# boelnasr/ManipulaPy

Hardware: AMD Instinct MI355X
Metric: joint-timesteps/sec (NxBxDOF) inverse-dynamics trajectory (higher is better)
Workload: dtype f32; 1 GPU; UR5 6-DOF, B=4096 x N=1000, inverse_dynamics_trajectory fp32 (BASELINE configs[1]); robot=ur5, dof=6, B_per_gpu=4096, N=1000, rows_per_gpu=4096000, op=id, inputs=q/qd/qdd histories resident in HBM, input_sets=3, bytes_between_reuse=1179648000, kernel_variant=robot-specialised (hiprtc)

## Files before the change

### manipulapy_amd/csrc/mp_core.h

```cpp
#pragma once

#if !defined(__HIPCC_RTC__)
#include <cmath>
#endif

#include "mp_model.h"

#if defined(__HIPCC__) || defined(__HIPCC_RTC__)
#define MP_HD __host__ __device__ __forceinline__
#else
#define MP_HD inline
#endif

#if defined(__clang__)
#define MP_HAS_PACKED 1
typedef float mp_f2 __attribute__((ext_vector_type(2)));
typedef int mp_i2 __attribute__((ext_vector_type(2)));
typedef unsigned mp_u2 __attribute__((ext_vector_type(2)));
#endif

template <typename T> struct MpTraits;
template <> struct MpTraits<float> {
  using S = float;
  static MP_HD float splat(float v) { return v; }
// ... 54 lines not shown
  c = __builtin_bit_cast(double, __builtin_bit_cast(unsigned long long, b) ^ ((unsigned long long)((qs + 0x40000000u) & 0x80000000u) << 32));
}
#if MP_HAS_PACKED
MP_HD void mp_sincos(mp_f2 x, mp_f2& s, mp_f2& c) {
  const mp_f2 kf = __builtin_elementwise_fma(x, (mp_f2)(0.636619772367581343f), (mp_f2)(12582912.0f));
  const mp_f2 k = kf - 12582912.0f;
  mp_f2 r = __builtin_elementwise_fma(-k, (mp_f2)(1.57079637050628662109375f), x);
  r = __builtin_elementwise_fma(-k, (mp_f2)(-4.37113900018624283e-8f), r);
  const mp_f2 r2 = r * r;
  mp_f2 ps = __builtin_elementwise_fma(r2, (mp_f2)(-1.9515295891e-4f), (mp_f2)(8.3321608736e-3f));
  ps = __builtin_elementwise_fma(r2, ps, (mp_f2)(-1.6666654611e-1f));
  ps = __builtin_elementwise_fma(r * r2, ps, r);
  mp_f2 pc = __builtin_elementwise_fma(r2, (mp_f2)(2.443315711809948e-5f), (mp_f2)(-1.388731625493765e-3f));
  pc = __builtin_elementwise_fma(r2, pc, (mp_f2)(4.166664568298827e-2f));
  pc = __builtin_elementwise_fma(r2 * r2, pc, __builtin_elementwise_fma(r2, (mp_f2)(-0.5f), (mp_f2)(1.0f)));
  const mp_i2 q = __builtin_bit_cast(mp_i2, kf);
  const mp_i2 odd = (q & 1) != 0;
  const mp_f2 a = odd ? pc : ps;
  const mp_f2 b = odd ? ps : pc;
  const mp_u2 qs = __builtin_bit_cast(mp_u2, q) << 30;
  s = __builtin_bit_cast(mp_f2, __builtin_bit_cast(mp_u2, a) ^ (qs & 0x80000000u));
  c = __builtin_bit_cast(mp_f2, __builtin_bit_cast(mp_u2, b) ^ ((qs + 0x40000000u) & 0x80000000u));
}
#endif

MP_HD float mp_min(float a, float b) { return a < b ? a : b; }
MP_HD float mp_max(float a, float b) { return a > b ? a : b; }
MP_HD double mp_min(double a, double b) { return a < b ? a : b; }
MP_HD double mp_max(double a, double b) { return a > b ? a : b; }
#if MP_HAS_PACKED
MP_HD mp_f2 mp_min(mp_f2 a, mp_f2 b) { return (a < b) ? a : b; }
MP_HD mp_f2 mp_max(mp_f2 a, mp_f2 b) { return (a > b) ? a : b; }
#endif
MP_HD float mp_abs(float a) { return __builtin_fabsf(a); }
MP_HD double mp_abs(double a) { return __builtin_fabs(a); }
#if MP_HAS_PACKED
MP_HD mp_f2 mp_abs(mp_f2 a) { return __builtin_elementwise_abs(a); }
#endif
MP_HD float mp_sqrt(float x) { return sqrtf(x); }
MP_HD double mp_sqrt(double x) { return sqrt(x); }
#if MP_HAS_PACKED
MP_HD mp_f2 mp_sqrt(mp_f2 x) { return (mp_f2){sqrtf(x.x), sqrtf(x.y)}; }
#endif
MP_HD float mp_rsqrt(float x) {
#if defined(__HIP_DEVICE_COMPILE__)
  const float y = __builtin_amdgcn_rsqf(x);
  const float e = fmaf(-(x * y), y, 1.0f);
  return fmaf(0.5f * y, e, y);
#else
  return 1.0f / sqrtf(x);
#endif
}
MP_HD double mp_rsqrt(double x) { return 1.0 / sqrt(x); }
#if MP_HAS_PACKED
MP_HD mp_f2 mp_rsqrt(mp_f2 x) { return (mp_f2){mp_rsqrt(x.x), mp_rsqrt(x.y)}; }
#endif
template <typename T>
MP_HD T mp_clip(T v, typename MpTraits<T>::S lo, typename MpTraits<T>::S hi) {
  return mp_min(mp_max(v, MpTraits<T>::splat(lo)), MpTraits<T>::splat(hi));
}

MP_HD int mp_hi_word(float x) { return __builtin_bit_cast(int, x); }
MP_HD int mp_hi_word(double x) { return (int)(__builtin_bit_cast(long long, x) >> 32); }
template <typename T> struct MpBadBits;
template <> struct MpBadBits<float> { static constexpr int POS = 0x7f800000; static constexpr unsigned NEG = 0xff800000u; };
template <> struct MpBadBits<double> { static constexpr int POS = 0x7ff00000; static constexpr unsigned NEG = 0xfff00000u; };

template <typename T>
struct MpBad {
  int ms = 0;
  unsigned mu = 0;
  MP_HD void add(T v) {
    const int b = mp_hi_word(v);
    ms = b > ms ? b : ms;
    mu = (unsigned)b > mu ? (unsigned)b : mu;
  }
  template <int N> MP_HD void add(const T (&v)[N]) {
#pragma unroll
    for (int i = 0; i < N; ++i) add(v[i]);
  }
  MP_HD bool any() const { return ms >= MpBadBits<T>::POS || mu >= MpBadBits<T>::NEG; }
};
MP_HD void mp_poison_if(bool bad, float& v) {
  const unsigned b = __builtin_bit_cast(unsigned, v);
  v = __builtin_bit_cast(float, bad ? 0x7fc00000u : b);
}
MP_HD void mp_poison_if(bool bad, double& v) {
  const unsigned long long b = __builtin_bit_cast(unsigned long long, v);
  v = __builtin_bit_cast(double, bad ? 0x7ff8000000000000ull : b);
}
#if MP_HAS_PACKED
template <>
struct MpBad<mp_f2> {
  MpBad<float> x, y;
  MP_HD void add(mp_f2 v) { x.add(v.x); y.add(v.y); }
  template <int N> MP_HD void add(const mp_f2 (&v)[N]) {
#pragma unroll
    for (int i = 0; i < N; ++i) add(v[i]);
  }
};
#endif
template <typename T, int N>
MP_HD void mp_poison_if(bool bad, T (&v)[N]) {
#pragma unroll
  for (int i = 0; i < N; ++i) mp_poison_if(bad, v[i]);
}

template <typename MT>
MP_HD const auto& mp_joint_of(const MT& M, int i) { return M.j[i]; }
#if defined(__HIP_DEVICE_COMPILE__)
typedef const __attribute__((address_space(4))) MpModel<float> MpModelConstF;
typedef const __attribute__((address_space(4))) MpModel<double> MpModelConstD;
__device__ __forceinline__ const __attribute__((address_space(4))) MpJoint<float>& mp_joint_of(MpModelConstF& M, int i) {
  MpModelConstF* p = &M;
  asm volatile("" : "+s"(p));
  return p->j[i];
}
__device__ __forceinline__ const __attribute__((address_space(4))) MpJoint<double>& mp_joint_of(MpModelConstD& M, int i) {
  MpModelConstD* p = &M;
  asm volatile("" : "+s"(p));
  return p->j[i];
}
typedef const __attribute__((address_space(4))) MpModelRev<float> MpModelRevConstF;
template <> struct MpAllRevolute<MpModelRevConstF> { static constexpr bool value = true; };
template <> struct MpAllRevolute<__attribute__((address_space(4))) MpModelRev<float>> { static constexpr bool value = true; };
__device__ __forceinline__ const __attribute__((address_space(4))) MpJoint<float>& mp_joint_of(MpModelRevConstF& M, int i) {
  MpModelRevConstF* p = &M;
  asm volatile("" : "+s"(p));
  return p->j[i];
}
#endif

template <typename T, typename S>
MP_HD void mp_motion_A(S ca, S sa, S a, T& wx, T& wy, T& wz, T& vx, T& vy, T& vz) {
  const T ty = vy + a * wz, tz = vz - a * wy;
  vy = ca * ty + sa * tz;
  vz = ca * tz - sa * ty;
  const T uy = wy;
  wy = ca * uy + sa * wz;
  wz = ca * wz - sa * uy;
  (void)wx; (void)vx;
}
template <typename T>
MP_HD void mp_motion_B(T c, T s, T d, T& wx, T& wy, T& wz, T& vx, T& vy, T& vz) {
  const T tx = vx + d * wy, ty = vy - d * wx;
  vx = c * tx + s * ty;
  vy = c * ty - s * tx;
  const T ux = wx;
  wx = c * ux + s * wy;
  wy = c * wy - s * ux;
  (void)wz; (void)vz;
}
template <typename T, typename S>
MP_HD void mp_force_down_A(S ca, S sa, S a, T& nx, T& ny, T& nz, T& fx, T& fy, T& fz) {
  const T ty = ny + a * fz, tz = nz - a * fy;
  ny = ca * ty + sa * tz;
  nz = ca * tz - sa * ty;
  const T uy = fy;
  fy = ca * uy + sa * fz;
  fz = ca * fz - sa * uy;
  (void)nx; (void)fx;
}
template <typename T>
MP_HD void mp_force_down_B(T c, T s, T d, T& nx, T& ny, T& nz, T& fx, T& fy, T& fz) {
  const T tx = nx + d * fy, ty = ny - d * fx;
  nx = c * tx + s * ty;
  ny = c * ty - s * tx;
  const T ux = fx;
  fx = c * ux + s * fy;
  fy = c * fy - s * ux;
  (void)nz; (void)fz;
}
template <typename T>
MP_HD void mp_force_up_B(T c, T s, T d, T& nx, T& ny, T& nz, T& fx, T& fy, T& fz) {
  const T gx = c * fx - s * fy, gy = s * fx + c * fy;
  const T mx = c * nx - s * ny, my = s * nx + c * ny;
  fx = gx; fy = gy;
  nx = mx - d * gy;
  ny = my + d * gx;
  (void)nz; (void)fz;
}
template <typename T, typename S>
MP_HD void mp_force_up_A(S ca, S sa, S a, T& nx, T& ny, T& nz, T& fx, T& fy, T& fz) {
  const T gy = ca * fy - sa * fz, gz = sa * fy + ca * fz;
  const T my = ca * ny - sa * nz, mz = sa * ny + ca * nz;
  fy = gy; fz = gz;
  ny = my - a * gz;
  nz = mz + a * gy;
  (void)nx; (void)fx;
}

template <typename T, int N>
struct MpJointState {
  T s[N], c[N], d[N];
};

template <typename T, int N, typename MT>
MP_HD void mp_joint_state(const MT& M, const T (&q)[N], MpJointState<T, N>& js) {
  constexpr bool kAllRev = MpAllRevolute<MT>::value;
#pragma unroll
  for (int i = 0; i < N; ++i) {
    const auto& J = mp_joint_of(M, i);
    const T qr = kAllRev ? q[i] : J.rev * q[i];
    T s0, c0;
    mp_sincos(qr, s0, c0);
    js.s[i] = s0 * J.co + c0 * J.so;
    js.c[i] = c0 * J.co - s0 * J.so;
    if (kAllRev) js.d[i] = MpTraits<T>::splat(J.d);
    else js.d[i] = J.d + (q[i] - qr);
  }
}

struct MpNoScale {
  template <typename T> MP_HD void joint(int, const T&, const T&, const T&, const T&, const T&, const T&) {}
  template <typename T> MP_HD void body(int, const T&, const T&, const T&, const T&, const T&, const T&) {}
  template <typename T> MP_HD void child(int, const T&, const T&, const T&, const T&, const T&, const T&) {}
};
template <typename T, int N>
struct MpRowScale {
  static constexpr int J = N > 1 ? 1 : 0;
  static constexpr int JF = N > 2 ? 2 : N - 1;
  T bm, cm, f;
  static MP_HD T inf3(const T& x, const T& y, const T& z) { return mp_max(mp_max(mp_abs(x), mp_abs(y)), mp_abs(z)); }
  MP_HD void body(int i, const T& nx, const T& ny, const T& nz, const T&, const T&, const T&) {
    if (i == J) bm = inf3(nx, ny, nz);
  }
  MP_HD void joint(int i, const T&, const T&, const T&, const T& fx, const T& fy, const T& fz) {
    if (i == JF) f = inf3(fx, fy, fz);
  }
  MP_HD void child(int i, const T& nx, const T& ny, const T& nz, const T&, const T&, const T&) {
    if (i == J + 1) cm = inf3(nx, ny, nz);
  }
  template <typename S> MP_HD T scale(S lscale) const {
    const T lf = f * MpTraits<T>::splat(lscale);
    if (N > J + 1) return mp_max(mp_max(bm, cm), lf);
    return mp_max(bm, lf);
  }
};
template <typename T, int N, bool HAS_FTIP, typename SC, typename MT>
MP_HD void mp_rnea_impl(const MT& M, const typename MpTraits<T>::S (&a0)[3], const T (&tipn)[3], const T (&tipf)[3],
                        const MpJointState<T, N>& js, const T (&qd)[N], const T (&qdd)[N], T (&tau)[N], SC& sc) {
  using S = typename MpTraits<T>::S;
  using TR = MpTraits<T>;
  const T zero = TR::splat(S(0));
  T fnx[N], fny[N], fnz[N], ffx[N], ffy[N], ffz[N];
  T wx = zero, wy = zero, wz = zero, vx = zero, vy = zero, vz = zero;
  T dwx = zero, dwy = zero, dwz = zero, dvx = TR::splat(a0[0]), dvy = TR::splat(a0[1]), dvz = TR::splat(a0[2]);
  T tnx = zero, tny = zero, tnz = zero, tfx = zero, tfy = zero, tfz = zero;
  if (HAS_FTIP) { tnx = tipn[0]; tny = tipn[1]; tnz = tipn[2]; tfx = tipf[0]; tfy = tipf[1]; tfz = tipf[2]; }

#pragma unroll
  for (int i = 0; i < N; ++i) {
    const auto& J = mp_joint_of(M, i);
    if (i > 0) {
      mp_motion_A(J.ca, J.sa, J.a, wx, wy, wz, vx, vy, vz);
      mp_motion_A(J.ca, J.sa, J.a, dwx, dwy, dwz, dvx, dvy, dvz);
      if (HAS_FTIP) mp_force_down_A(J.ca, J.sa, J.a, tnx, tny, tnz, tfx, tfy, tfz);
    }
    const T c = js.c[i], s = js.s[i], d = js.d[i];
    mp_motion_B(c, s, d, wx, wy, wz, vx, vy, vz);
    mp_motion_B(c, s, d, dwx, dwy, dwz, dvx, dvy, dvz);
    if (HAS_FTIP) mp_force_down_B(c, s, d, tnx, tny, tnz, tfx, tfy, tfz);

    if (MpAllRevolute<MT>::value) {
      const T qdr = qd[i], ar = qdd[i];
      wz += qdr;
      dwx += qdr * wy;
      dwy -= qdr * wx;
      dwz += ar;
      dvx += qdr * vy;
      dvy -= qdr * vx;
    } else {
      const T qdr = J.rev * qd[i], qdp = qd[i] - qdr;
      const T ar = J.rev * qdd[i], ap = qdd[i] - ar;
      wz += qdr;
      vz += qdp;
      dwx += qdr * wy;
      dwy -= qdr * wx;
      dwz += ar;
      dvx += qdr * vy + qdp * wy;
      dvy -= qdr * vx + qdp * wx;
      dvz += ap;
    }

    const T pnx = J.Ixx * wx + J.Ixy * wy + J.Ixz * wz + (J.hy * vz - J.hz * vy);
    const T pny = J.Ixy * wx + J.Iyy * wy + J.Iyz * wz + (J.hz * vx - J.hx * vz);
    const T pnz = J.Ixz * wx + J.Iyz * wy + J.Izz * wz + (J.hx * vy - J.hy * vx);
    const T pfx = J.m * vx - (J.hy * wz - J.hz * wy);
    const T pfy = J.m * vy - (J.hz * wx - J.hx * wz);
    const T pfz = J.m * vz - (J.hx * wy - J.hy * wx);
    fnx[i] = J.Ixx * dwx + J.Ixy * dwy + J.Ixz * dwz + (J.hy * dvz - J.hz * dvy) + (wy * pnz - wz * pny) + (vy * pfz - vz * pfy);
    fny[i] = J.Ixy * dwx + J.Iyy * dwy + J.Iyz * dwz + (J.hz * dvx - J.hx * dvz) + (wz * pnx - wx * pnz) + (vz * pfx - vx * pfz);
    fnz[i] = J.Ixz * dwx + J.Iyz * dwy + J.Izz * dwz + (J.hx * dvy - J.hy * dvx) + (wx * pny - wy * pnx) + (vx * pfy - vy * pfx);
    ffx[i] = J.m * dvx - (J.hy * dwz - J.hz * dwy) + (wy * pfz - wz * pfy);
    ffy[i] = J.m * dvy - (J.hz * dwx - J.hx * dwz) + (wz * pfx - wx * pfz);
    ffz[i] = J.m * dvz - (J.hx * dwy - J.hy * dwx) + (wx * pfy - wy * pfx);
    sc.body(i, fnx[i], fny[i], fnz[i], ffx[i], ffy[i], ffz[i]);
  }
  if (HAS_FTIP) {
    fnx[N - 1] += tnx; fny[N - 1] += tny; fnz[N - 1] += tnz;
    ffx[N - 1] += tfx; ffy[N - 1] += tfy; ffz[N - 1] += tfz;
  }
#pragma unroll
  for (int i = N - 1; i >= 0; --i) {
    const auto& J = mp_joint_of(M, i);
    if (MpAllRevolute<MT>::value) tau[i] = fnz[i];
    else tau[i] = J.rev * fnz[i] + (S(1) - J.rev) * ffz[i];
    sc.joint(i, fnx[i], fny[i], fnz[i], ffx[i], ffy[i], ffz[i]);
    if (i > 0) {
      T nx = fnx[i], ny = fny[i], nz = fnz[i], fx = ffx[i], fy = ffy[i], fz = ffz[i];
      mp_force_up_B(js.c[i], js.s[i], js.d[i], nx, ny, nz, fx, fy, fz);
      mp_force_up_A(J.ca, J.sa, J.a, nx, ny, nz, fx, fy, fz);
      sc.child(i, nx, ny, nz, fx, fy, fz);
      fnx[i - 1] += nx; fny[i - 1] += ny; fnz[i - 1] += nz;
      ffx[i - 1] += fx; ffy[i - 1] += fy; ffz[i - 1] += fz;
    }
  }
}

template <typename T, int N, bool HAS_FTIP, typename MT>
MP_HD void mp_rnea(const MT& M, const typename MpTraits<T>::S (&a0)[3], const T (&tipn)[3], const T (&tipf)[3],
                   const MpJointState<T, N>& js, const T (&qd)[N], const T (&qdd)[N], T (&tau)[N]) {
  MpNoScale sc;
  mp_rnea_impl<T, N, HAS_FTIP>(M, a0, tipn, tipf, js, qd, qdd, tau, sc);
}

template <typename T, int N, bool HAS_FTIP, typename MT>
MP_HD void mp_rnea(const MT& M, const MpCall<typename MpTraits<T>::S>& C, const MpJointState<T, N>& js,
                   const T (&qd)[N], const T (&qdd)[N], T (&tau)[N]) {
  using TR = MpTraits<T>;
  const T tn[3] = {TR::splat(C.F1n[0]), TR::splat(C.F1n[1]), TR::splat(C.F1n[2])};
  const T tf[3] = {TR::splat(C.F1f[0]), TR::splat(C.F1f[1]), TR::splat(C.F1f[2])};
  mp_rnea<T, N, HAS_FTIP>(M, C.a0, tn, tf, js, qd, qdd, tau);
}

#ifndef MP_HARD_ROW_K
#define MP_HARD_ROW_K 8.0f
#endif
#ifndef MP_ADAPTIVE_F32
#define MP_ADAPTIVE_F32 1
#endif
template <int N>
MP_HD bool mp_id_row_is_hard(const float (&tau)[N], float scale) {
  float rowmax = mp_abs(tau[0]);
#pragma unroll
  for (int i = 1; i < N; ++i) rowmax = mp_max(rowmax, mp_abs(tau[i]));
  return scale > MP_HARD_ROW_K * rowmax;
}

template <int N, bool HAS_FTIP, typename MT>
MP_HD bool mp_rnea_f32(const MT& M, const MpCall<float>& C, const MpJointState<float, N>& js, const float (&qd)[N],
                       const float (&qdd)[N], float (&tau)[N]) {
#if MP_ADAPTIVE_F32
  const float tn[3] = {C.F1n[0], C.F1n[1], C.F1n[2]}, tf[3] = {C.F1f[0], C.F1f[1], C.F1f[2]};
  MpRowScale<float, N> sc;
  mp_rnea_impl<float, N, HAS_FTIP>(M, C.a0, tn, tf, js, qd, qdd, tau, sc);
  return mp_id_row_is_hard<N>(tau, sc.scale(M.lscale));
#else
  mp_rnea<float, N, HAS_FTIP>(M, C, js, qd, qdd, tau);
  return false;
#endif
}

template <int N> struct MpColdSlot { static constexpr int BYTES = 8 * N * 8 + 4 * N * 4; };
template <int N>
struct MpColdLocal {
  double f[8 * N];
  float j[4 * N];
  MP_HD double getf(int k) const { return f[k]; }
  MP_HD void putf(int k, double v) { f[k] = v; }
  MP_HD float getj(int k) const { return j[k]; }
  MP_HD void putj(int k, float v) { j[k] = v; }
};
#if defined(__HIP_DEVICE_COMPILE__)
#define MP_LDS_AS __attribute__((address_space(3)))
#else
#define MP_LDS_AS
#endif
template <int N>
struct MpColdMem {
  MP_LDS_AS char* p;
  MP_HD double getf(int k) const { return reinterpret_cast<const volatile MP_LDS_AS double*>(p)[k]; }
  MP_HD void putf(int k, double v) { reinterpret_cast<volatile MP_LDS_AS double*>(p)[k] = v; }
  MP_HD float getj(int k) const { return reinterpret_cast<const volatile MP_LDS_AS float*>(p + 8 * N * 8)[k]; }
  MP_HD void putj(int k, float v) { reinterpret_cast<volatile MP_LDS_AS float*>(p + 8 * N * 8)[k] = v; }
};

#if defined(__clang__)
#define MP_ROLLED _Pragma("clang loop unroll(disable)")
#else
#define MP_ROLLED
#endif
#if defined(__HIP_DEVICE_COMPILE__)
#define MP_STAGE() __builtin_amdgcn_sched_barrier(0)
#else
#define MP_STAGE() ((void)0)
#endif
template <int N, bool HAS_FTIP, typename MT, typename ST>
MP_HD void mp_rnea_cold(const MT& M, const MpCall<float>& C, const float (&q)[N], const float (&qd)[N], const float (&qdd)[N], ST st,
                        float (&tau)[N]) {
  double wx = 0, wy = 0, wz = 0, vx = 0, vy = 0, vz = 0;
  double dwx = 0, dwy = 0, dwz = 0, dvx = (double)C.a0[0], dvy = (double)C.a0[1], dvz = (double)C.a0[2];
  double tnx = 0, tny = 0, tnz = 0, tfx = 0, tfy = 0, tfz = 0;
  if (HAS_FTIP) { tnx = (double)C.F1n[0]; tny = (double)C.F1n[1]; tnz = (double)C.F1n[2]; tfx = (double)C.F1f[0]; tfy = (double)C.F1f[1]; tfz = (double)C.F1f[2]; }
#pragma unroll
  for (int i = 0; i < N; ++i) { st.putj(N + i, q[i]); st.putj(2 * N + i, qd[i]); st.putj(3 * N + i, qdd[i]); }
  MP_ROLLED
  for (int i = 0; i < N; ++i) {
    const auto& J = mp_joint_of(M, i);
    const float qi = st.getj(N + i);
    double s, c, d;
    {
      const double qr = (double)J.rev * (double)qi;
      double s0, c0;
      mp_sincos(qr, s0, c0);
      s = s0 * (double)J.co + c0 * (double)J.so;
      c = c0 * (double)J.co - s0 * (double)J.so;
      d = (double)J.d + ((double)qi - qr);
      st.putf(6 * N + i, s); st.putf(7 * N + i, c); st.putj(i, (float)d);
    }
    MP_STAGE();
    const double ca = (double)J.ca, sa = (double)J.sa, la = (double)J.a;
    if (i > 0) {
      mp_motion_A<double, double>(ca, sa, la, wx, wy, wz, vx, vy, vz);
      mp_motion_A<double, double>(ca, sa, la, dwx, dwy, dwz, dvx, dvy, dvz);
      if (HAS_FTIP) mp_force_down_A<double, double>(ca, sa, la, tnx, tny, tnz, tfx, tfy, tfz);
    }
    mp_motion_B<double>(c, s, d, wx, wy, wz, vx, vy, vz);
    mp_motion_B<double>(c, s, d, dwx, dwy, dwz, dvx, dvy, dvz);
    if (HAS_FTIP) mp_force_down_B<double>(c, s, d, tnx, tny, tnz, tfx, tfy, tfz);
    const double rev = (double)J.rev, qdi = (double)st.getj(2 * N + i), qddi = (double)st.getj(3 * N + i);
    const double qdr = rev * qdi, qdp = qdi - qdr;
    const double ar = rev * qddi, ap = qddi - ar;
    wz += qdr;
    vz += qdp;
    dwx += qdr * wy;
    dwy -= qdr * wx;
    dwz += ar;
    dvx += qdr * vy + qdp * wy;
    dvy -= qdr * vx + qdp * wx;
    dvz += ap;
    MP_STAGE();
    const double Ixx = (double)J.Ixx, Ixy = (double)J.Ixy, Ixz = (double)J.Ixz, Iyy = (double)J.Iyy, Iyz = (double)J.Iyz, Izz = (double)J.Izz;
    const double hx = (double)J.hx, hy = (double)J.hy, hz = (double)J.hz, m = (double)J.m;
    const double pnx = Ixx * wx + Ixy * wy + Ixz * wz + (hy * vz - hz * vy);
    const double pny = Ixy * wx + Iyy * wy + Iyz * wz + (hz * vx - hx * vz);
    const double pnz = Ixz * wx + Iyz * wy + Izz * wz + (hx * vy - hy * vx);
    const double pfx = m * vx - (hy * wz - hz * wy);
    const double pfy = m * vy - (hz * wx - hx * wz);
    const double pfz = m * vz - (hx * wy - hy * wx);
    MP_STAGE();
    st.putf(6 * i + 0, Ixx * dwx + Ixy * dwy + Ixz * dwz + (hy * dvz - hz * dvy) + (wy * pnz - wz * pny) + (vy * pfz - vz * pfy));
    MP_STAGE();
    st.putf(6 * i + 1, Ixy * dwx + Iyy * dwy + Iyz * dwz + (hz * dvx - hx * dvz) + (wz * pnx - wx * pnz) + (vz * pfx - vx * pfz));
    MP_STAGE();
    st.putf(6 * i + 2, Ixz * dwx + Iyz * dwy + Izz * dwz + (hx * dvy - hy * dvx) + (wx * pny - wy * pnx) + (vx * pfy - vy * pfx));
    MP_STAGE();
    st.putf(6 * i + 3, m * dvx - (hy * dwz - hz * dwy) + (wy * pfz - wz * pfy));
    st.putf(6 * i + 4, m * dvy - (hz * dwx - hx * dwz) + (wz * pfx - wx * pfz));
    st.putf(6 * i + 5, m * dvz - (hx * dwy - hy * dwx) + (wx * pfy - wy * pfx));
    MP_STAGE();
  }
  double ax = tnx, ay = tny, az = tnz, bx = tfx, by = tfy, bz = tfz;
  MP_ROLLED
  for (int i = N - 1; i >= 0; --i) {
    const auto& J = mp_joint_of(M, i);
    double nx = st.getf(6 * i + 0) + ax, ny = st.getf(6 * i + 1) + ay, nz = st.getf(6 * i + 2) + az;
    double fx = st.getf(6 * i + 3) + bx, fy = st.getf(6 * i + 4) + by, fz = st.getf(6 * i + 5) + bz;
    const double rev = (double)J.rev;
    st.putj(N + i, (float)(rev * nz + (1.0 - rev) * fz));
    if (i > 0) {
      const double s = st.getf(6 * N + i), c = st.getf(7 * N + i), d = (double)st.getj(i);
      mp_force_up_B<double>(c, s, d, nx, ny, nz, fx, fy, fz);
      mp_force_up_A<double, double>((double)J.ca, (double)J.sa, (double)J.a, nx, ny, nz, fx, fy, fz);
      ax = nx; ay = ny; az = nz; bx = fx; by = fy; bz = fz;
    }
  }
#pragma unroll
  for (int i = 0; i < N; ++i) tau[i] = st.getj(N + i);
}

template <typename T> struct MpIsF32 { static constexpr bool value = false; };
template <> struct MpIsF32<float> { static constexpr bool value = true; };
template <typename T, int N, bool HAS_FTIP, typename MT>
MP_HD void mp_rnea_row(const MT& M, const MpCall<typename MpTraits<T>::S>& C, const MpJointState<T, N>& js, const T (&q)[N],
                       const T (&qd)[N], const T (&qdd)[N], T (&tau)[N]) {
  if constexpr (MpIsF32<T>::value) {
    if (mp_rnea_f32<N, HAS_FTIP>(M, C, js, qd, qdd, tau)) {
      MpColdLocal<N> st;
      if (C.cold_model) mp_rnea_cold<N, HAS_FTIP>(*static_cast<const MpModel<double>*>(C.cold_model), C, q, qd, qdd, st, tau);
      else mp_rnea_cold<N, HAS_FTIP>(M, C, q, qd, qdd, st, tau);
    }
  } else {
    mp_rnea<T, N, HAS_FTIP>(M, C, js, qd, qdd, tau);
  }
}

template <typename T, typename MT>
MP_HD void mp_wrench_to_frame1(const MT& M, const T (&F)[6], T (&tn)[3], T (&tf)[3]) {
  const auto& R = M.base_R;
  const auto& p = M.base_p;
  const T nx = F[0] - (p[1] * F[5] - p[2] * F[4]), ny = F[1] - (p[2] * F[3] - p[0] * F[5]), nz = F[2] - (p[0] * F[4] - p[1] * F[3]);
#pragma unroll
  for (int k = 0; k < 3; ++k) {
    tn[k] = R[0 + k] * nx + R[3 + k] * ny + R[6 + k] * nz;
    tf[k] = R[0 + k] * F[3] + R[3 + k] * F[4] + R[6 + k] * F[5];
  }
}

template <typename T, int N, typename MT>
MP_HD void mp_mass_matrix(const MT& M, const MpJointState<T, N>& js, T (&Mq)[N][N]) {
  using S = typename MpTraits<T>::S;
  using TR = MpTraits<T>;
  const S a0[3] = {S(0), S(0), S(0)};
  const T zero = TR::splat(S(0));
  const T z3[3] = {zero, zero, zero};
  T col[N][N];
#pragma unroll
  for (int j = 0; j < N; ++j) {
    T qd[N], qdd[N];
#pragma unroll
    for (int k = 0; k < N; ++k) { qd[k] = zero; qdd[k] = (k == j) ? TR::splat(S(1)) : zero; }
    mp_rnea<T, N, false>(M, a0, z3, z3, js, qd, qdd, col[j]);
  }
#pragma unroll
  for (int i = 0; i < N; ++i)
#pragma unroll
    for (int j = 0; j < N; ++j) Mq[i][j] = S(0.5) * (col[j][i] + col[i][j]);
}

template <typename T>
struct MpRbi {
  T m, hx, hy, hz, xx, xy, xz, yy, yz, zz;
};

template <typename T>
MP_HD void mp_rbi_up_B(T c, T s, T d, MpRbi<T>& I) {
  const T hx = c * I.hx - s * I.hy, hy = s * I.hx + c * I.hy;
  const T cc = c * c, ss = s * s, sc = s * c;
  const T xx = cc * I.xx - (sc + sc) * I.xy + ss * I.yy;
  const T yy = ss * I.xx + (sc + sc) * I.xy + cc * I.yy;
  const T xy = sc * (I.xx - I.yy) + (cc - ss) * I.xy;
  const T xz = c * I.xz - s * I.yz, yz = s * I.xz + c * I.yz;
  const T t = d * (I.hz + I.hz) + I.m * d * d;
  I.xx = xx + t; I.yy = yy + t; I.xy = xy;
  I.xz = xz - d * hx; I.yz = yz - d * hy;
  I.hx = hx; I.hy = hy; I.hz = I.hz + I.m * d;
}
template <typename T, typename S>
MP_HD void mp_rbi_up_A(S ca, S sa, S a, MpRbi<T>& I) {
  const T hy = ca * I.hy - sa * I.hz, hz = sa * I.hy + ca * I.hz;
  const S cc = ca * ca, ss = sa * sa, sc = sa * ca;
  const T yy = cc * I.yy - (sc + sc) * I.yz + ss * I.zz;
  const T zz = ss * I.yy + (sc + sc) * I.yz + cc * I.zz;
  const T yz = sc * (I.yy - I.zz) + (cc - ss) * I.yz;
  const T xy = ca * I.xy - sa * I.xz, xz = sa * I.xy + ca * I.xz;
  const T t = a * (I.hx + I.hx) + I.m * (a * a);
  I.yy = yy + t; I.zz = zz + t; I.yz = yz;
  I.xy = xy - a * hy; I.xz = xz - a * hz;
  I.hy = hy; I.hz = hz; I.hx = I.hx + I.m * a;
}

template <typename T, int N, typename MT>
MP_HD void mp_mass_matrix_crba(const MT& M, const MpJointState<T, N>& js, T (&Mq)[N][N]) {
  using S = typename MpTraits<T>::S;
  using TR = MpTraits<T>;
  const T zero = TR::splat(S(0));
  MpRbi<T> Ic;
  Ic.m = zero; Ic.hx = zero; Ic.hy = zero; Ic.hz = zero;
  Ic.xx = zero; Ic.xy = zero; Ic.xz = zero; Ic.yy = zero; Ic.yz = zero; Ic.zz = zero;
#pragma unroll
  for (int i = N - 1; i >= 0; --i) {
    const auto& J = mp_joint_of(M, i);
    Ic.m = Ic.m + J.m; Ic.hx = Ic.hx + J.hx; Ic.hy = Ic.hy + J.hy; Ic.hz = Ic.hz + J.hz;
    Ic.xx = Ic.xx + J.Ixx; Ic.xy = Ic.xy + J.Ixy; Ic.xz = Ic.xz + J.Ixz; Ic.yy = Ic.yy + J.Iyy; Ic.yz = Ic.yz + J.Iyz;
    Ic.zz = Ic.zz + J.Izz;
    const S r = J.rev, p = S(1) - J.rev;
    T nx = r * Ic.xz + p * Ic.hy, ny = r * Ic.yz - p * Ic.hx, nz = r * Ic.zz;
    T fx = -(r * Ic.hy), fy = r * Ic.hx, fz = p * Ic.m;
    Mq[i][i] = r * nz + p * fz;
#pragma unroll
    for (int k = i; k > 0; --k) {
      const auto& Jk = mp_joint_of(M, k);
      mp_force_up_B(js.c[k], js.s[k], js.d[k], nx, ny, nz, fx, fy, fz);
      mp_force_up_A(Jk.ca, Jk.sa, Jk.a, nx, ny, nz, fx, fy, fz);
      const auto& Jp = mp_joint_of(M, k - 1);
      const T v = Jp.rev * nz + (S(1) - Jp.rev) * fz;
      Mq[k - 1][i] = v;
      Mq[i][k - 1] = v;
    }
    if (i > 0) {
      mp_rbi_up_B(js.c[i], js.s[i], js.d[i], Ic);
      mp_rbi_up_A(J.ca, J.sa, J.a, Ic);
    }
  }
}

template <typename T, int N>
MP_HD void mp_spd_solve(T (&A)[N][N], T (&b)[N]) {
#pragma unroll
  for (int j = 0; j < N; ++j) {
    T d = A[j][j];
#pragma unroll
    for (int k = 0; k < j; ++k) d -= A[j][k] * A[j][k];
    const T inv = mp_rsqrt(d);
    A[j][j] = inv;
#pragma unroll
    for (int i = j + 1; i < N; ++i) {
      T v = A[i][j];
#pragma unroll
      for (int k = 0; k < j; ++k) v -= A[i][k] * A[j][k];
      A[i][j] = v * inv;
    }
  }
#pragma unroll
  for (int i = 0; i < N; ++i) {
    T v = b[i];
#pragma unroll
    for (int k = 0; k < i; ++k) v -= A[i][k] * b[k];
    b[i] = v * A[i][i];
  }
#pragma unroll
  for (int i = N - 1; i >= 0; --i) {
    T v = b[i];
#pragma unroll
    for (int k = i + 1; k < N; ++k) v -= A[k][i] * b[k];
    b[i] = v * A[i][i];
  }
// ... 189 lines not shown
```

### manipulapy_amd/csrc/mp_dyn.h

```cpp
#pragma once

#include "mp_core.h"

#if defined(__clang__)
#define MP_NOUNROLL _Pragma("nounroll")
#else
#define MP_NOUNROLL
#endif

template <typename T, int CAP>
struct MpDynState {
  T s[CAP], c[CAP], d[CAP];
};

template <typename T, typename MT, int CAP>
MP_HD void mp_dyn_joint_state(const MT& M, int n, const T* q, MpDynState<T, CAP>& js) {
  MP_NOUNROLL
  for (int i = 0; i < n; ++i) {
    const auto& J = M.j[i];
    const T qr = J.rev * q[i];
    T s0, c0;
    mp_sincos(qr, s0, c0);
    js.s[i] = s0 * J.co + c0 * J.so;
    js.c[i] = c0 * J.co - s0 * J.so;
    js.d[i] = J.d + (q[i] - qr);
  }
}

template <typename T, bool HAS_FTIP, typename MT, int CAP>
MP_HD void mp_dyn_rnea(const MT& M, int n, const T (&a0)[3], const T (&tipn)[3], const T (&tipf)[3], const MpDynState<T, CAP>& js,
                       const T* qd, const T* qdd, T* tau, T* scale = nullptr) {
  const int sJ = n > 1 ? 1 : 0, sJF = n > 2 ? 2 : n - 1;
  T s_bm = 0, s_cm = 0, s_f = 0;
  T fnx[CAP], fny[CAP], fnz[CAP], ffx[CAP], ffy[CAP], ffz[CAP];
  T wx = 0, wy = 0, wz = 0, vx = 0, vy = 0, vz = 0;
  T dwx = 0, dwy = 0, dwz = 0, dvx = a0[0], dvy = a0[1], dvz = a0[2];
  T tnx = 0, tny = 0, tnz = 0, tfx = 0, tfy = 0, tfz = 0;
  if (HAS_FTIP) { tnx = tipn[0]; tny = tipn[1]; tnz = tipn[2]; tfx = tipf[0]; tfy = tipf[1]; tfz = tipf[2]; }
  MP_NOUNROLL
  for (int i = 0; i < n; ++i) {
    const auto& J = M.j[i];
    if (i > 0) {
      mp_motion_A(J.ca, J.sa, J.a, wx, wy, wz, vx, vy, vz);
      mp_motion_A(J.ca, J.sa, J.a, dwx, dwy, dwz, dvx, dvy, dvz);
      if (HAS_FTIP) mp_force_down_A(J.ca, J.sa, J.a, tnx, tny, tnz, tfx, tfy, tfz);
    }
    const T c = js.c[i], s = js.s[i], d = js.d[i];
    mp_motion_B(c, s, d, wx, wy, wz, vx, vy, vz);
    mp_motion_B(c, s, d, dwx, dwy, dwz, dvx, dvy, dvz);
    if (HAS_FTIP) mp_force_down_B(c, s, d, tnx, tny, tnz, tfx, tfy, tfz);
    const T qdr = J.rev * qd[i], qdp = qd[i] - qdr;
    const T ar = J.rev * qdd[i], ap = qdd[i] - ar;
    wz += qdr;
    vz += qdp;
    dwx += qdr * wy;
    dwy -= qdr * wx;
    dwz += ar;
    dvx += qdr * vy + qdp * wy;
    dvy -= qdr * vx + qdp * wx;
    dvz += ap;
    const T pnx = J.Ixx * wx + J.Ixy * wy + J.Ixz * wz + (J.hy * vz - J.hz * vy);
    const T pny = J.Ixy * wx + J.Iyy * wy + J.Iyz * wz + (J.hz * vx - J.hx * vz);
    const T pnz = J.Ixz * wx + J.Iyz * wy + J.Izz * wz + (J.hx * vy - J.hy * vx);
    const T pfx = J.m * vx - (J.hy * wz - J.hz * wy);
    const T pfy = J.m * vy - (J.hz * wx - J.hx * wz);
    const T pfz = J.m * vz - (J.hx * wy - J.hy * wx);
    fnx[i] = J.Ixx * dwx + J.Ixy * dwy + J.Ixz * dwz + (J.hy * dvz - J.hz * dvy) + (wy * pnz - wz * pny) + (vy * pfz - vz * pfy);
    fny[i] = J.Ixy * dwx + J.Iyy * dwy + J.Iyz * dwz + (J.hz * dvx - J.hx * dvz) + (wz * pnx - wx * pnz) + (vz * pfx - vx * pfz);
    fnz[i] = J.Ixz * dwx + J.Iyz * dwy + J.Izz * dwz + (J.hx * dvy - J.hy * dvx) + (wx * pny - wy * pnx) + (vx * pfy - vy * pfx);
    ffx[i] = J.m * dvx - (J.hy * dwz - J.hz * dwy) + (wy * pfz - wz * pfy);
    ffy[i] = J.m * dvy - (J.hz * dwx - J.hx * dwz) + (wz * pfx - wx * pfz);
    ffz[i] = J.m * dvz - (J.hx * dwy - J.hy * dwx) + (wx * pfy - wy * pfx);
    if (scale && i == sJ) s_bm = mp_max(mp_max(mp_abs(fnx[i]), mp_abs(fny[i])), mp_abs(fnz[i]));
  }
  if (HAS_FTIP) {
    fnx[n - 1] += tnx; fny[n - 1] += tny; fnz[n - 1] += tnz;
    ffx[n - 1] += tfx; ffy[n - 1] += tfy; ffz[n - 1] += tfz;
  }
  MP_NOUNROLL
  for (int i = n - 1; i >= 0; --i) {
    const auto& J = M.j[i];
    tau[i] = J.rev * fnz[i] + (T(1) - J.rev) * ffz[i];
    if (scale && i == sJF) s_f = mp_max(mp_max(mp_abs(ffx[i]), mp_abs(ffy[i])), mp_abs(ffz[i]));
    if (i > 0) {
      T nx = fnx[i], ny = fny[i], nz = fnz[i], fx = ffx[i], fy = ffy[i], fz = ffz[i];
      mp_force_up_B(js.c[i], js.s[i], js.d[i], nx, ny, nz, fx, fy, fz);
      mp_force_up_A(J.ca, J.sa, J.a, nx, ny, nz, fx, fy, fz);
      if (scale && i == sJ + 1) s_cm = mp_max(mp_max(mp_abs(nx), mp_abs(ny)), mp_abs(nz));
      fnx[i - 1] += nx; fny[i - 1] += ny; fnz[i - 1] += nz;
      ffx[i - 1] += fx; ffy[i - 1] += fy; ffz[i - 1] += fz;
    }
  }
  if (scale) *scale = mp_max(mp_max(s_bm, s_cm), s_f * (T)M.lscale);
}

#if defined(__HIP_DEVICE_COMPILE__)
typedef const __attribute__((address_space(4))) MpBigModel<double> MpBigConstD;
#else
typedef const MpBigModel<double> MpBigConstD;
#endif
MP_HD bool mp_dyn_row_is_hard(const float* tau, int n, float scale) {
  float rowmax = 0.0f;
  for (int i = 0; i < n; ++i) rowmax = mp_max(rowmax, mp_abs(tau[i]));
  return scale > MP_HARD_ROW_K * rowmax;
}
template <int CAP, bool HAS_FTIP>
MP_HD void mp_dyn_row_id_f64(MpBigConstD& Md, const MpCall<float>& C, const float* q, const float* qd, const float* qdd, float* tau) {
  const int n = Md.n;
  double a[CAP], b[CAP], c[CAP], t[CAP];
  for (int j = 0; j < n; ++j) { a[j] = (double)q[j]; b[j] = (double)qd[j]; c[j] = (double)qdd[j]; }
  const double a0[3] = {(double)C.a0[0], (double)C.a0[1], (double)C.a0[2]};
  const double tn[3] = {(double)C.F1n[0], (double)C.F1n[1], (double)C.F1n[2]}, tf[3] = {(double)C.F1f[0], (double)C.F1f[1], (double)C.F1f[2]};
  MpDynState<double, CAP> js;
  mp_dyn_joint_state<double>(Md, n, a, js);
  mp_dyn_rnea<double, HAS_FTIP>(Md, n, a0, tn, tf, js, b, c, t);
  for (int j = 0; j < n; ++j) tau[j] = (float)t[j];
}

template <typename T, typename MT, int CAP>
MP_HD void mp_dyn_mass_matrix(const MT& M, int n, const MpDynState<T, CAP>& js, T* Mq, int ld) {
  MpRbi<T> Ic;
  Ic.m = 0; Ic.hx = 0; Ic.hy = 0; Ic.hz = 0; Ic.xx = 0; Ic.xy = 0; Ic.xz = 0; Ic.yy = 0; Ic.yz = 0; Ic.zz = 0;
  MP_NOUNROLL
  for (int i = n - 1; i >= 0; --i) {
    const auto& J = M.j[i];
    Ic.m = Ic.m + J.m; Ic.hx = Ic.hx + J.hx; Ic.hy = Ic.hy + J.hy; Ic.hz = Ic.hz + J.hz;
    Ic.xx = Ic.xx + J.Ixx; Ic.xy = Ic.xy + J.Ixy; Ic.xz = Ic.xz + J.Ixz; Ic.yy = Ic.yy + J.Iyy; Ic.yz = Ic.yz + J.Iyz;
    Ic.zz = Ic.zz + J.Izz;
    const T r = J.rev, p = T(1) - J.rev;
    T nx = r * Ic.xz + p * Ic.hy, ny = r * Ic.yz - p * Ic.hx, nz = r * Ic.zz;
    T fx = -(r * Ic.hy), fy = r * Ic.hx, fz = p * Ic.m;
    Mq[i * ld + i] = r * nz + p * fz;
    MP_NOUNROLL
    for (int k = i; k > 0; --k) {
      const auto& Jk = M.j[k];
      mp_force_up_B(js.c[k], js.s[k], js.d[k], nx, ny, nz, fx, fy, fz);
      mp_force_up_A(Jk.ca, Jk.sa, Jk.a, nx, ny, nz, fx, fy, fz);
      const T rp = M.j[k - 1].rev;
      const T v = rp * nz + (T(1) - rp) * fz;
      Mq[(k - 1) * ld + i] = v;
      Mq[i * ld + (k - 1)] = v;
    }
    if (i > 0) {
      mp_rbi_up_B(js.c[i], js.s[i], js.d[i], Ic);
      mp_rbi_up_A(J.ca, J.sa, J.a, Ic);
    }
  }
}

template <typename T>
MP_HD void mp_dyn_spd_solve(int n, T* A, int ld, T* b) {
  MP_NOUNROLL
  for (int j = 0; j < n; ++j) {
    T d = A[j * ld + j];
    for (int k = 0; k < j; ++k) d -= A[j * ld + k] * A[j * ld + k];
    const T inv = mp_rsqrt(d);
    A[j * ld + j] = inv;
    for (int i = j + 1; i < n; ++i) {
      T v = A[i * ld + j];
      for (int k = 0; k < j; ++k) v -= A[i * ld + k] * A[j * ld + k];
      A[i * ld + j] = v * inv;
    }
  }
  MP_NOUNROLL
  for (int i = 0; i < n; ++i) {
    T v = b[i];
    for (int k = 0; k < i; ++k) v -= A[i * ld + k] * b[k];
    b[i] = v * A[i * ld + i];
  }
  MP_NOUNROLL
  for (int i = n - 1; i >= 0; --i) {
    T v = b[i];
    for (int k = i + 1; k < n; ++k) v -= A[k * ld + i] * b[k];
    b[i] = v * A[i * ld + i];
  }
}

template <int CAP, typename T, bool HAS_FTIP, typename MT>
MP_HD void mp_dyn_forward_dynamics(const MT& M, int n, const T (&a0)[3], const T (&tipn)[3], const T (&tipf)[3], const T* q,
                                   const T* qd, const T* tau, T* qdd) {
  MpDynState<T, CAP> js;
  mp_dyn_joint_state<T>(M, n, q, js);
  T zero[CAP], bias[CAP], Mq[CAP * CAP];
  for (int k = 0; k < n; ++k) zero[k] = T(0);
  mp_dyn_rnea<T, HAS_FTIP>(M, n, a0, tipn, tipf, js, qd, zero, bias);
  mp_dyn_mass_matrix<T>(M, n, js, Mq, CAP);
  for (int k = 0; k < n; ++k) qdd[k] = tau[k] - bias[k];
  mp_dyn_spd_solve<T>(n, Mq, CAP, qdd);
}

template <typename T, typename MT, int CAP>
MP_HD void mp_dyn_fk_jac(const MT& M, int n, const MpDynState<T, CAP>& js, T* Tout, T* Jout) {
  T x0 = M.base_R[0], x1 = M.base_R[3], x2 = M.base_R[6];
  T y0 = M.base_R[1], y1 = M.base_R[4], y2 = M.base_R[7];
  T z0 = M.base_R[2], z1 = M.base_R[5], z2 = M.base_R[8];
  T p0 = M.base_p[0], p1 = M.base_p[1], p2 = M.base_p[2];
  MP_NOUNROLL
  for (int i = 0; i < n; ++i) {
    const auto& J = M.j[i];
    if (i > 0) {
      p0 += J.a * x0; p1 += J.a * x1; p2 += J.a * x2;
      const T a0 = y0, a1 = y1, a2 = y2;
      y0 = J.ca * a0 + J.sa * z0; y1 = J.ca * a1 + J.sa * z1; y2 = J.ca * a2 + J.sa * z2;
      z0 = J.ca * z0 - J.sa * a0; z1 = J.ca * z1 - J.sa * a1; z2 = J.ca * z2 - J.sa * a2;
    }
    if (Jout) {
      const T cx = p1 * z2 - p2 * z1, cy = p2 * z0 - p0 * z2, cz = p0 * z1 - p1 * z0;
      const T r = J.rev, pr = T(1) - J.rev;
      Jout[0 * n + i] = r * z0; Jout[1 * n + i] = r * z1; Jout[2 * n + i] = r * z2;
      Jout[3 * n + i] = r * cx + pr * z0; Jout[4 * n + i] = r * cy + pr * z1; Jout[5 * n + i] = r * cz + pr * z2;
    }
    const T c = js.c[i], s = js.s[i], d = js.d[i];
    const T b0 = x0, b1 = x1, b2 = x2;
    x0 = c * b0 + s * y0; x1 = c * b1 + s * y1; x2 = c * b2 + s * y2;
    y0 = c * y0 - s * b0; y1 = c * y1 - s * b1; y2 = c * y2 - s * b2;
    p0 += d * z0; p1 += d * z1; p2 += d * z2;
  }
  if (Tout) {
    const auto& R = M.tool_R;
    const auto& t = M.tool_p;
    Tout[0] = x0 * R[0] + y0 * R[3] + z0 * R[6]; Tout[1] = x0 * R[1] + y0 * R[4] + z0 * R[7]; Tout[2] = x0 * R[2] + y0 * R[5] + z0 * R[8];
    Tout[4] = x1 * R[0] + y1 * R[3] + z1 * R[6]; Tout[5] = x1 * R[1] + y1 * R[4] + z1 * R[7]; Tout[6] = x1 * R[2] + y1 * R[5] + z1 * R[8];
    Tout[8] = x2 * R[0] + y2 * R[3] + z2 * R[6]; Tout[9] = x2 * R[1] + y2 * R[4] + z2 * R[7]; Tout[10] = x2 * R[2] + y2 * R[5] + z2 * R[8];
    Tout[3] = p0 + x0 * t[0] + y0 * t[1] + z0 * t[2];
    Tout[7] = p1 + x1 * t[0] + y1 * t[1] + z1 * t[2];
// ... 186 lines not shown
```

Baseline: 385.7 billion joint-timesteps/s.

## Reformulate RNEA forward pass with classical origin acceleration instead of spatial velocity

Drops the linear velocity state and tracks the classical origin acceleration directly. New combined transform helpers propagate omega, its derivative, and the linear acceleration together, and the body force formulas are simplified to avoid computing momentum terms. This cuts ALU work and register pressure in the hot per-joint loop of the specialised, cold-path and dynamic kernels. It risks small numerical differences from the reordered floating-point operations.

```diff
diff --git a/manipulapy_amd/csrc/mp_core.h b/manipulapy_amd/csrc/mp_core.h
--- a/manipulapy_amd/csrc/mp_core.h
+++ b/manipulapy_amd/csrc/mp_core.h
@@ -230,6 +230,32 @@
   (void)wz; (void)vz;
 }
 template <typename T, typename S>
+MP_HD void mp_accel_A(S ca, S sa, S l, T& wx, T& wy, T& wz, T& dwx, T& dwy, T& dwz, T& ax, T& ay, T& az) {
+  ax = ax - l * (wy * wy + wz * wz);
+  const T ty = ay + l * (dwz + wx * wy), tz = az - l * (dwy - wx * wz);
+  ay = ca * ty + sa * tz;
+  az = ca * tz - sa * ty;
+  const T ey = dwy;
+  dwy = ca * ey + sa * dwz;
+  dwz = ca * dwz - sa * ey;
+  const T uy = wy;
+  wy = ca * uy + sa * wz;
+  wz = ca * wz - sa * uy;
+}
+template <typename T>
+MP_HD void mp_accel_B(T c, T s, T d, T& wx, T& wy, T& wz, T& dwx, T& dwy, T& dwz, T& ax, T& ay, T& az) {
+  const T tx = ax + d * (dwy + wx * wz), ty = ay - d * (dwx - wy * wz);
+  az = az - d * (wx * wx + wy * wy);
+  ax = c * tx + s * ty;
+  ay = c * ty - s * tx;
+  const T ex = dwx;
+  dwx = c * ex + s * dwy;
+  dwy = c * dwy - s * ex;
+  const T ux = wx;
+  wx = c * ux + s * wy;
+  wy = c * wy - s * ux;
+}
+template <typename T, typename S>
 MP_HD void mp_force_down_A(S ca, S sa, S a, T& nx, T& ny, T& nz, T& fx, T& fy, T& fz) {
   const T ty = ny + a * fz, tz = nz - a * fy;
   ny = ca * ty + sa * tz;
@@ -322,8 +348,8 @@
   using TR = MpTraits<T>;
   const T zero = TR::splat(S(0));
   T fnx[N], fny[N], fnz[N], ffx[N], ffy[N], ffz[N];
-  T wx = zero, wy = zero, wz = zero, vx = zero, vy = zero, vz = zero;
-  T dwx = zero, dwy = zero, dwz = zero, dvx = TR::splat(a0[0]), dvy = TR::splat(a0[1]), dvz = TR::splat(a0[2]);
+  T wx = zero, wy = zero, wz = zero;
+  T dwx = zero, dwy = zero, dwz = zero, ax = TR::splat(a0[0]), ay = TR::splat(a0[1]), az = TR::splat(a0[2]);
   T tnx = zero, tny = zero, tnz = zero, tfx = zero, tfy = zero, tfz = zero;
   if (HAS_FTIP) { tnx = tipn[0]; tny = tipn[1]; tnz = tipn[2]; tfx = tipf[0]; tfy = tipf[1]; tfz = tipf[2]; }
 
@@ -331,13 +357,11 @@
   for (int i = 0; i < N; ++i) {
     const auto& J = mp_joint_of(M, i);
     if (i > 0) {
-      mp_motion_A(J.ca, J.sa, J.a, wx, wy, wz, vx, vy, vz);
-      mp_motion_A(J.ca, J.sa, J.a, dwx, dwy, dwz, dvx, dvy, dvz);
+      mp_accel_A(J.ca, J.sa, J.a, wx, wy, wz, dwx, dwy, dwz, ax, ay, az);
       if (HAS_FTIP) mp_force_down_A(J.ca, J.sa, J.a, tnx, tny, tnz, tfx, tfy, tfz);
     }
     const T c = js.c[i], s = js.s[i], d = js.d[i];
-    mp_motion_B(c, s, d, wx, wy, wz, vx, vy, vz);
-    mp_motion_B(c, s, d, dwx, dwy, dwz, dvx, dvy, dvz);
+    mp_accel_B(c, s, d, wx, wy, wz, dwx, dwy, dwz, ax, ay, az);
     if (HAS_FTIP) mp_force_down_B(c, s, d, tnx, tny, tnz, tfx, tfy, tfz);
 
     if (MpAllRevolute<MT>::value) {
@@ -346,33 +370,29 @@
       dwx += qdr * wy;
       dwy -= qdr * wx;
       dwz += ar;
-      dvx += qdr * vy;
-      dvy -= qdr * vx;
     } else {
       const T qdr = J.rev * qd[i], qdp = qd[i] - qdr;
       const T ar = J.rev * qdd[i], ap = qdd[i] - ar;
+      const T qdp2 = qdp + qdp;
       wz += qdr;
-      vz += qdp;
       dwx += qdr * wy;
       dwy -= qdr * wx;
       dwz += ar;
-      dvx += qdr * vy + qdp * wy;
-      dvy -= qdr * vx + qdp * wx;
-      dvz += ap;
-    }
-
-    const T pnx = J.Ixx * wx + J.Ixy * wy + J.Ixz * wz + (J.hy * vz - J.hz * vy);
-    const T pny = J.Ixy * wx + J.Iyy * wy + J.Iyz * wz + (J.hz * vx - J.hx * vz);
-    const T pnz = J.Ixz * wx + J.Iyz * wy + J.Izz * wz + (J.hx * vy - J.hy * vx);
-    const T pfx = J.m * vx - (J.hy * wz - J.hz * wy);
-    const T pfy = J.m * vy - (J.hz * wx - J.hx * wz);
-    const T pfz = J.m * vz - (J.hx * wy - J.hy * wx);
-    fnx[i] = J.Ixx * dwx + J.Ixy * dwy + J.Ixz * dwz + (J.hy * dvz - J.hz * dvy) + (wy * pnz - wz * pny) + (vy * pfz - vz * pfy);
-    fny[i] = J.Ixy * dwx + J.Iyy * dwy + J.Iyz * dwz + (J.hz * dvx - J.hx * dvz) + (wz * pnx - wx * pnz) + (vz * pfx - vx * pfz);
-    fnz[i] = J.Ixz * dwx + J.Iyz * dwy + J.Izz * dwz + (J.hx * dvy - J.hy * dvx) + (wx * pny - wy * pnx) + (vx * pfy - vy * pfx);
-    ffx[i] = J.m * dvx - (J.hy * dwz - J.hz * dwy) + (wy * pfz - wz * pfy);
-    ffy[i] = J.m * dvy - (J.hz * dwx - J.hx * dwz) + (wz * pfx - wx * pfz);
-    ffz[i] = J.m * dvz - (J.hx * dwy - J.hy * dwx) + (wx * pfy - wy * pfx);
+      ax += qdp2 * wy;
+      ay -= qdp2 * wx;
+      az += ap;
+    }
+
+    const T iwx = J.Ixx * wx + J.Ixy * wy + J.Ixz * wz;
+    const T iwy = J.Ixy * wx + J.Iyy * wy + J.Iyz * wz;
+    const T iwz = J.Ixz * wx + J.Iyz * wy + J.Izz * wz;
+    const T ux = J.hy * wz - J.hz * wy, uy = J.hz * wx - J.hx * wz, uz = J.hx * wy - J.hy * wx;
+    fnx[i] = J.Ixx * dwx + J.Ixy * dwy + J.Ixz * dwz + (J.hy * az - J.hz * ay) + (wy * iwz - wz * iwy);
+    fny[i] = J.Ixy * dwx + J.Iyy * dwy + J.Iyz * dwz + (J.hz * ax - J.hx * az) + (wz * iwx - wx * iwz);
+    fnz[i] = J.Ixz * dwx + J.Iyz * dwy + J.Izz * dwz + (J.hx * ay - J.hy * ax) + (wx * iwy - wy * iwx);
+    ffx[i] = J.m * ax - (J.hy * dwz - J.hz * dwy) - (wy * uz - wz * uy);
+    ffy[i] = J.m * ay - (J.hz * dwx - J.hx * dwz) - (wz * ux - wx * uz);
+    ffz[i] = J.m * az - (J.hx * dwy - J.hy * dwx) - (wx * uy - wy * ux);
     sc.body(i, fnx[i], fny[i], fnz[i], ffx[i], ffy[i], ffz[i]);
   }
   if (HAS_FTIP) {
@@ -477,8 +497,8 @@
 template <int N, bool HAS_FTIP, typename MT, typename ST>
 MP_HD void mp_rnea_cold(const MT& M, const MpCall<float>& C, const float (&q)[N], const float (&qd)[N], const float (&qdd)[N], ST st,
                         float (&tau)[N]) {
-  double wx = 0, wy = 0, wz = 0, vx = 0, vy = 0, vz = 0;
-  double dwx = 0, dwy = 0, dwz = 0, dvx = (double)C.a0[0], dvy = (double)C.a0[1], dvz = (double)C.a0[2];
+  double wx = 0, wy = 0, wz = 0, dwx = 0, dwy = 0, dwz = 0;
+  double ax = (double)C.a0[0], ay = (double)C.a0[1], az = (double)C.a0[2];
   double tnx = 0, tny = 0, tnz = 0, tfx = 0, tfy = 0, tfz = 0;
   if (HAS_FTIP) { tnx = (double)C.F1n[0]; tny = (double)C.F1n[1]; tnz = (double)C.F1n[2]; tfx = (double)C.F1f[0]; tfy = (double)C.F1f[1]; tfz = (double)C.F1f[2]; }
 #pragma unroll
@@ -500,58 +520,53 @@
     MP_STAGE();
     const double ca = (double)J.ca, sa = (double)J.sa, la = (double)J.a;
     if (i > 0) {
-      mp_motion_A<double, double>(ca, sa, la, wx, wy, wz, vx, vy, vz);
-      mp_motion_A<double, double>(ca, sa, la, dwx, dwy, dwz, dvx, dvy, dvz);
+      mp_accel_A<double, double>(ca, sa, la, wx, wy, wz, dwx, dwy, dwz, ax, ay, az);
       if (HAS_FTIP) mp_force_down_A<double, double>(ca, sa, la, tnx, tny, tnz, tfx, tfy, tfz);
     }
-    mp_motion_B<double>(c, s, d, wx, wy, wz, vx, vy, vz);
-    mp_motion_B<double>(c, s, d, dwx, dwy, dwz, dvx, dvy, dvz);
+    mp_accel_B<double>(c, s, d, wx, wy, wz, dwx, dwy, dwz, ax, ay, az);
     if (HAS_FTIP) mp_force_down_B<double>(c, s, d, tnx, tny, tnz, tfx, tfy, tfz);
     const double rev = (double)J.rev, qdi = (double)st.getj(2 * N + i), qddi = (double)st.getj(3 * N + i);
-    const double qdr = rev * qdi, qdp = qdi - qdr;
+    const double qdr = rev * qdi, qdp2 = 2.0 * (qdi - qdr);
     const double ar = rev * qddi, ap = qddi - ar;
     wz += qdr;
-    vz += qdp;
     dwx += qdr * wy;
     dwy -= qdr * wx;
     dwz += ar;
-    dvx += qdr * vy + qdp * wy;
-    dvy -= qdr * vx + qdp * wx;
-    dvz += ap;
+    ax += qdp2 * wy;
+    ay -= qdp2 * wx;
+    az += ap;
     MP_STAGE();
     const double Ixx = (double)J.Ixx, Ixy = (double)J.Ixy, Ixz = (double)J.Ixz, Iyy = (double)J.Iyy, Iyz = (double)J.Iyz, Izz = (double)J.Izz;
     const double hx = (double)J.hx, hy = (double)J.hy, hz = (double)J.hz, m = (double)J.m;
-    const double pnx = Ixx * wx + Ixy * wy + Ixz * wz + (hy * vz - hz * vy);
-    const double pny = Ixy * wx + Iyy * wy + Iyz * wz + (hz * vx - hx * vz);
-    const double pnz = Ixz * wx + Iyz * wy + Izz * wz + (hx * vy - hy * vx);
-    const double pfx = m * vx - (hy * wz - hz * wy);
-    const double pfy = m * vy - (hz * wx - hx * wz);
-    const double pfz = m * vz - (hx * wy - hy * wx);
+    const double iwx = Ixx * wx + Ixy * wy + Ixz * wz;
+    const double iwy = Ixy * wx + Iyy * wy + Iyz * wz;
+    const double iwz = Ixz * wx + Iyz * wy + Izz * wz;
+    const double ux = hy * wz - hz * wy, uy = hz * wx - hx * wz, uz = hx * wy - hy * wx;
     MP_STAGE();
-    st.putf(6 * i + 0, Ixx * dwx + Ixy * dwy + Ixz * dwz + (hy * dvz - hz * dvy) + (wy * pnz - wz * pny) + (vy * pfz - vz * pfy));
+    st.putf(6 * i + 0, Ixx * dwx + Ixy * dwy + Ixz * dwz + (hy * az - hz * ay) + (wy * iwz - wz * iwy));
     MP_STAGE();
-    st.putf(6 * i + 1, Ixy * dwx + Iyy * dwy + Iyz * dwz + (hz * dvx - hx * dvz) + (wz * pnx - wx * pnz) + (vz * pfx - vx * pfz));
+    st.putf(6 * i + 1, Ixy * dwx + Iyy * dwy + Iyz * dwz + (hz * ax - hx * az) + (wz * iwx - wx * iwz));
     MP_STAGE();
-    st.putf(6 * i + 2, Ixz * dwx + Iyz * dwy + Izz * dwz + (hx * dvy - hy * dvx) + (wx * pny - wy * pnx) + (vx * pfy - vy * pfx));
+    st.putf(6 * i + 2, Ixz * dwx + Iyz * dwy + Izz * dwz + (hx * ay - hy * ax) + (wx * iwy - wy * iwx));
     MP_STAGE();
-    st.putf(6 * i + 3, m * dvx - (hy * dwz - hz * dwy) + (wy * pfz - wz * pfy));
-    st.putf(6 * i + 4, m * dvy - (hz * dwx - hx * dwz) + (wz * pfx - wx * pfz));
-    st.putf(6 * i + 5, m * dvz - (hx * dwy - hy * dwx) + (wx * pfy - wy * pfx));
+    st.putf(6 * i + 3, m * ax - (hy * dwz - hz * dwy) - (wy * uz - wz * uy));
+    st.putf(6 * i + 4, m * ay - (hz * dwx - hx * dwz) - (wz * ux - wx * uz));
+    st.putf(6 * i + 5, m * az - (hx * dwy - hy * dwx) - (wx * uy - wy * ux));
     MP_STAGE();
   }
-  double ax = tnx, ay = tny, az = tnz, bx = tfx, by = tfy, bz = tfz;
+  double cnx = tnx, cny = tny, cnz = tnz, cfx = tfx, cfy = tfy, cfz = tfz;
   MP_ROLLED
   for (int i = N - 1; i >= 0; --i) {
     const auto& J = mp_joint_of(M, i);
-    double nx = st.getf(6 * i + 0) + ax, ny = st.getf(6 * i + 1) + ay, nz = st.getf(6 * i + 2) + az;
-    double fx = st.getf(6 * i + 3) + bx, fy = st.getf(6 * i + 4) + by, fz = st.getf(6 * i + 5) + bz;
+    double nx = st.getf(6 * i + 0) + cnx, ny = st.getf(6 * i + 1) + cny, nz = st.getf(6 * i + 2) + cnz;
+    double fx = st.getf(6 * i + 3) + cfx, fy = st.getf(6 * i + 4) + cfy, fz = st.getf(6 * i + 5) + cfz;
     const double rev = (double)J.rev;
     st.putj(N + i, (float)(rev * nz + (1.0 - rev) * fz));
     if (i > 0) {
       const double s = st.getf(6 * N + i), c = st.getf(7 * N + i), d = (double)st.getj(i);
       mp_force_up_B<double>(c, s, d, nx, ny, nz, fx, fy, fz);
       mp_force_up_A<double, double>((double)J.ca, (double)J.sa, (double)J.a, nx, ny, nz, fx, fy, fz);
-      ax = nx; ay = ny; az = nz; bx = fx; by = fy; bz = fz;
+      cnx = nx; cny = ny; cnz = nz; cfx = fx; cfy = fy; cfz = fz;
     }
   }
 #pragma unroll
diff --git a/manipulapy_amd/csrc/mp_dyn.h b/manipulapy_amd/csrc/mp_dyn.h
--- a/manipulapy_amd/csrc/mp_dyn.h
+++ b/manipulapy_amd/csrc/mp_dyn.h
@@ -33,44 +33,39 @@
   const int sJ = n > 1 ? 1 : 0, sJF = n > 2 ? 2 : n - 1;
   T s_bm = 0, s_cm = 0, s_f = 0;
   T fnx[CAP], fny[CAP], fnz[CAP], ffx[CAP], ffy[CAP], ffz[CAP];
-  T wx = 0, wy = 0, wz = 0, vx = 0, vy = 0, vz = 0;
-  T dwx = 0, dwy = 0, dwz = 0, dvx = a0[0], dvy = a0[1], dvz = a0[2];
+  T wx = 0, wy = 0, wz = 0, dwx = 0, dwy = 0, dwz = 0;
+  T ax = a0[0], ay = a0[1], az = a0[2];
   T tnx = 0, tny = 0, tnz = 0, tfx = 0, tfy = 0, tfz = 0;
   if (HAS_FTIP) { tnx = tipn[0]; tny = tipn[1]; tnz = tipn[2]; tfx = tipf[0]; tfy = tipf[1]; tfz = tipf[2]; }
   MP_NOUNROLL
   for (int i = 0; i < n; ++i) {
     const auto& J = M.j[i];
     if (i > 0) {
-      mp_motion_A(J.ca, J.sa, J.a, wx, wy, wz, vx, vy, vz);
-      mp_motion_A(J.ca, J.sa, J.a, dwx, dwy, dwz, dvx, dvy, dvz);
+      mp_accel_A(J.ca, J.sa, J.a, wx, wy, wz, dwx, dwy, dwz, ax, ay, az);
       if (HAS_FTIP) mp_force_down_A(J.ca, J.sa, J.a, tnx, tny, tnz, tfx, tfy, tfz);
     }
     const T c = js.c[i], s = js.s[i], d = js.d[i];
-    mp_motion_B(c, s, d, wx, wy, wz, vx, vy, vz);
-    mp_motion_B(c, s, d, dwx, dwy, dwz, dvx, dvy, dvz);
+    mp_accel_B(c, s, d, wx, wy, wz, dwx, dwy, dwz, ax, ay, az);
     if (HAS_FTIP) mp_force_down_B(c, s, d, tnx, tny, tnz, tfx, tfy, tfz);
-    const T qdr = J.rev * qd[i], qdp = qd[i] - qdr;
+    const T qdr = J.rev * qd[i], qdp2 = T(2) * (qd[i] - qdr);
     const T ar = J.rev * qdd[i], ap = qdd[i] - ar;
     wz += qdr;
-    vz += qdp;
     dwx += qdr * wy;
     dwy -= qdr * wx;
     dwz += ar;
-    dvx += qdr * vy + qdp * wy;
-    dvy -= qdr * vx + qdp * wx;
-    dvz += ap;
-    const T pnx = J.Ixx * wx + J.Ixy * wy + J.Ixz * wz + (J.hy * vz - J.hz * vy);
-    const T pny = J.Ixy * wx + J.Iyy * wy + J.Iyz * wz + (J.hz * vx - J.hx * vz);
-    const T pnz = J.Ixz * wx + J.Iyz * wy + J.Izz * wz + (J.hx * vy - J.hy * vx);
-    const T pfx = J.m * vx - (J.hy * wz - J.hz * wy);
-    const T pfy = J.m * vy - (J.hz * wx - J.hx * wz);
-    const T pfz = J.m * vz - (J.hx * wy - J.hy * wx);
-    fnx[i] = J.Ixx * dwx + J.Ixy * dwy + J.Ixz * dwz + (J.hy * dvz - J.hz * dvy) + (wy * pnz - wz * pny) + (vy * pfz - vz * pfy);
-    fny[i] = J.Ixy * dwx + J.Iyy * dwy + J.Iyz * dwz + (J.hz * dvx - J.hx * dvz) + (wz * pnx - wx * pnz) + (vz * pfx - vx * pfz);
-    fnz[i] = J.Ixz * dwx + J.Iyz * dwy + J.Izz * dwz + (J.hx * dvy - J.hy * dvx) + (wx * pny - wy * pnx) + (vx * pfy - vy * pfx);
-    ffx[i] = J.m * dvx - (J.hy * dwz - J.hz * dwy) + (wy * pfz - wz * pfy);
-    ffy[i] = J.m * dvy - (J.hz * dwx - J.hx * dwz) + (wz * pfx - wx * pfz);
-    ffz[i] = J.m * dvz - (J.hx * dwy - J.hy * dwx) + (wx * pfy - wy * pfx);
+    ax += qdp2 * wy;
+    ay -= qdp2 * wx;
+    az += ap;
+    const T iwx = J.Ixx * wx + J.Ixy * wy + J.Ixz * wz;
+    const T iwy = J.Ixy * wx + J.Iyy * wy + J.Iyz * wz;
+    const T iwz = J.Ixz * wx + J.Iyz * wy + J.Izz * wz;
+    const T ux = J.hy * wz - J.hz * wy, uy = J.hz * wx - J.hx * wz, uz = J.hx * wy - J.hy * wx;
+    fnx[i] = J.Ixx * dwx + J.Ixy * dwy + J.Ixz * dwz + (J.hy * az - J.hz * ay) + (wy * iwz - wz * iwy);
+    fny[i] = J.Ixy * dwx + J.Iyy * dwy + J.Iyz * dwz + (J.hz * ax - J.hx * az) + (wz * iwx - wx * iwz);
+    fnz[i] = J.Ixz * dwx + J.Iyz * dwy + J.Izz * dwz + (J.hx * ay - J.hy * ax) + (wx * iwy - wy * iwx);
+    ffx[i] = J.m * ax - (J.hy * dwz - J.hz * dwy) - (wy * uz - wz * uy);
+    ffy[i] = J.m * ay - (J.hz * dwx - J.hx * dwz) - (wz * ux - wx * uz);
+    ffz[i] = J.m * az - (J.hx * dwy - J.hy * dwx) - (wx * uy - wy * ux);
     if (scale && i == sJ) s_bm = mp_max(mp_max(mp_abs(fnx[i]), mp_abs(fny[i])), mp_abs(fnz[i]));
   }
   if (HAS_FTIP) {
```

Result: no change. 389.3 billion joint-timesteps/s, median of 6 (+0.9%).
